# verlab/accelerated_features

Measured on AMD Instinct MI355X. Metric: frames/sec detectAndCompute+match (VGA, top_k=4096), higher is better.
Workload: dtype f32; 1 GPU; VGA 640x480 sparse top_k=4096, batch=64 per GPU: detectAndCompute + MNN match of the 32 consecutive frame pairs (BASELINE configs[1]); batch_per_gpu=64, height=480, width=640, top_k=4096, weights=synthetic (tests/fixtures.py), barrier=none (one rank), concurrent_lanes=True, lanes=2

## Files before the change

accelerated_features_amd/_lib.py:

```python
import ctypes as C
import os

_HERE = os.path.dirname(os.path.abspath(__file__))
LIB_PATH = os.environ.get("XFH_LIB_PATH") or os.path.join(_HERE, "libxfeat_hip.so")

XFH_OK = 0
LAYOUT_NCHW, LAYOUT_NHWC = 0, 1
LG_NO_PRUNING = 1 << 30
GUIDE_FUNDAMENTAL, GUIDE_HOMOGRAPHY = 0, 1
SAMPLE_MODES = {'nearest': 0, 'bilinear': 1, 'bicubic': 2}
PROF_NONE, PROF_CONV_MFMA, PROF_MATCH, PROF_BLOCK1, PROF_HEADS, PROF_CONV_64_64_S1, PROF_CONV_24_24, PROF_CONV_LAYER0 = 0, 1, 2, 3, 4, 5, 6, 100
PROF_ALL = 1000

_p = C.c_void_p
_i = C.c_int
_f = C.c_float
_sz = C.c_size_t
SIGNATURES = {
    "xfh_version": (_i, []),
    "xfh_last_error": (C.c_char_p, []),
    "xfh_num_weight_arrays": (_i, []),
    "xfh_weight_array_floats": (_sz, [_i]),
    "xfh_create": (_i, [C.POINTER(_p), _i, _i, C.POINTER(_p)]),
    "xfh_destroy": (None, [_p]),
    "xfh_resize_bilinear": (_i, [_p, _i, _i, _i, _p, _i, _i, _f, _f, _p]),
    "xfh_backbone_workspace_bytes": (_sz, [_i, _i, _i, _i]),
    "xfh_backbone": (_i, [_p, _p, _i, _i, _i, _i, _p, _p, _p, _p, _p, _p, _sz, _p]),
    "xfh_backbone_u8": (_i, [_p, _p, _i, _f, _i, _i, _i, _i, _p, _p, _p, _p, _p, _p, _sz, _p]),
    "xfh_backbone_resized": (_i, [_p, _p, _i, _i, _i, _i, _i, _i, _f, _f, _i, _i, _f, _f, _p, _p, _p, _p, _p, _p, _sz, _p]),
    "xfh_conv_layer": (_i, [_p, _i, _p, _i, _i, _i, _p, _i, _p]),
    "xfh_detect_workspace_bytes": (_sz, [_i, _i, _i, _i, _i]),
    "xfh_detect_sparse": (_i, [_p, _p, _p, _p, _p, _i, _i, _i, _f, _i, _i, _f, _f, _p, _p, _p, _p, _p, _p, _p, _sz, _p]),
    "xfh_dense_workspace_bytes": (_sz, [_i, _i, _i, _i]),
    "xfh_extract_dense": (_i, [_p, _p, _p, _i, _i, _i, _i, _f, _f, _f, _p, _p, _p, _p, _sz, _p]),
    "xfh_match_workspace_bytes": (_sz, [_i, _i, _i]),
# ... 107 lines not shown
```

accelerated_features_amd/csrc/api.hip:

```cpp
#include "../../include/xfeat_hip.h"
#include "kernels.hpp"
#include "weight_split.hpp"
#include "block1_fx.hpp"

#include <cmath>
#include <cstdarg>
#include <cstdio>
#include <cstring>
#include <vector>

using namespace xfh;

static thread_local char g_err[512] = "";
static int fail(int code, const char* fmt, ...) {
    va_list ap;
    va_start(ap, fmt);
    vsnprintf(g_err, sizeof(g_err), fmt, ap);
    va_end(ap);
    return code;
}
int xfh_set_error(int code, const char* fmt, ...) {
    char buf[512];
    va_list ap;
    va_start(ap, fmt);
// ... 222 lines not shown

int xfh_version(void) { return XFH_VERSION; }
const char* xfh_last_error(void) { return g_err; }
int xfh_num_weight_arrays(void) { return num_arrays(); }
size_t xfh_weight_array_floats(int i) { return array_floats(i); }

int xfh_create(const float* const* host_arrays, int n_arrays, int device, xfh_handle* out) {
    if (!host_arrays || !out) return fail(XFH_ERR_ARG, "xfh_create: NULL argument");
    if (n_arrays != num_arrays()) return fail(XFH_ERR_WEIGHTS, "xfh_create: expected %d weight arrays, got %d", num_arrays(), n_arrays);
    for (int i = 0; i < n_arrays; ++i)
        if (!host_arrays[i]) return fail(XFH_ERR_WEIGHTS, "xfh_create: weight array %d is NULL", i);
    int ndev = 0;
    if (hipGetDeviceCount(&ndev) != hipSuccess || ndev <= 0) return fail(XFH_ERR_DEVICE, "xfh_create: no HIP device visible");
    if (device < 0 || device >= ndev) return fail(XFH_ERR_DEVICE, "xfh_create: device %d out of range (%d visible)", device, ndev);
    hipDeviceProp_t prop;
    HIP_TRY(hipGetDeviceProperties(&prop, device));
    if (strncmp(prop.gcnArchName, "gfx950", 6) != 0)
        return fail(XFH_ERR_DEVICE, "xfh_create: device %d is %s; this library is built for gfx950 only", device, prop.gcnArchName);
    HIP_TRY(hipSetDevice(device));

    std::vector<float> blob;
    auto reserve = [&](size_t n) { size_t o = align_up(blob.size(), 64); blob.resize(o + n, 0.f); return o; };
    const size_t zoff = reserve(256);
    struct Off { size_t oihw, kc, kcp, bias, fx, rs; bool has_fx, has_rs; } coff[L_NUM];
    struct FOff { size_t w, b, fx; bool fx_ok; } foff[5];
    int ai = 0;
    for (int li = 0; li < L_NUM; ++li) {
        const ConvSpec& c = kConvs[li];
        const int kk = c.ks * c.ks, cpad = (c.cout + 31) / 32 * 32;
        const float* w = host_arrays[ai++];
        std::vector<double> scale(c.cout, 1.0), shift(c.cout, 0.0);
        if (c.bn) {
            const float* rm = host_arrays[ai++];
            const float* rv = host_arrays[ai++];
            for (int o = 0; o < c.cout; ++o) {
                if (!(rv[o] + kBnEps > 0)) return fail(XFH_ERR_WEIGHTS, "layer %d: running_var[%d] = %g is not positive", li, o, rv[o]);
                scale[o] = 1.0 / std::sqrt((double)rv[o] + kBnEps);
                shift[o] = -(double)rm[o] * scale[o];
            }
        } else {
            const float* b = host_arrays[ai++];
            for (int o = 0; o < c.cout; ++o) shift[o] = b[o];
        }
        coff[li].oihw = reserve((size_t)c.cout * c.cin * kk);
        coff[li].kc = reserve((size_t)c.cin * kk * c.cout);
        coff[li].kcp = reserve((size_t)c.cin * kk * cpad);
        coff[li].bias = reserve(cpad);
// ... 34 lines not shown
                    for (int lane = 0; lane < 64; ++lane) {
                        const int o = lane & 31, kg = 2 * st + (lane >> 5);
                        for (int i = 0; i < 8; ++i) {
                            float v = 0.f;
                            if (o < c.cout && kg < 9 * cg) v = blob[coff[li].oihw + ((size_t)o * c.cin + (kg % cg) * 8 + i) * 9 + kg / cg];
                            split_weight(v, q);
                            for (int sp = 0; sp < 3; ++sp) dst[(((size_t)st * 3 + sp) * 64 + lane) * 8 + i] = q[sp];
                        }
                    }
            if (bx24s2)
                for (int cb = 0; cb < 2; ++cb)
                    for (int st = 0; st < nstep; ++st)
                        for (int lane = 0; lane < 64; ++lane) {
                            const int o = cb * 32 + (lane & 31), kg = 2 * st + (lane >> 5);
                            for (int i = 0; i < 8; ++i) {
                                float v = 0.f;
                                if (kg < 9 * cg) v = blob[coff[li].oihw + ((size_t)o * c.cin + (kg % cg) * 8 + i) * 9 + kg / cg];
                                split_weight(v, q);
                                for (int sp = 0; sp < 3; ++sp) dst[((((size_t)cb * nstep + st) * 3 + sp) * 64 + lane) * 8 + i] = q[sp];
                            }
                        }
            if (bx64s2) pack_bx64(&blob[coff[li].oihw], c.cin, c.cout, dst);
        }
        coff[li].has_rs = false;
        if (bx1x1 && fx_ok) {
            coff[li].rs = reserve((size_t)4 * 2 * 3 * 64 * 4);
            pack_rs64_1x1(&blob[coff[li].oihw], reinterpret_cast<uint16_t*>(&blob[coff[li].rs]));
            coff[li].has_rs = true;
        }
        if (bx128 && fx_ok) {
            coff[li].rs = reserve(4 * kRs64Halfs / 2);
            pack_rs128(&blob[coff[li].oihw], reinterpret_cast<uint16_t*>(&blob[coff[li].rs]));
            coff[li].has_rs = true;
        }
        if (bx64 && fx_ok) {
            coff[li].rs = reserve(kRs64Halfs / 2);
            pack_rs64(&blob[coff[li].oihw], reinterpret_cast<uint16_t*>(&blob[coff[li].rs]));
            coff[li].has_rs = true;
        }
    }
    size_t head_off[2] = {0, 0}, head_boff[2] = {0, 0};
    bool head_fx_ok[2] = {true, true};
    const float head_b_last = blob[coff[L_HEAT_2].bias];
    {
        const int kp[4] = {L_KP_0, L_KP_1, L_KP_2, L_KP_3}, rel[2] = {L_HEAT_0, L_HEAT_1};
        for (int hd = 0; hd < 2; ++hd) {
// ... 65 lines not shown
            pack_linear_fx(wk.data(), f.k, npad, reinterpret_cast<uint16_t*>(blob.data() + foff[fi].fx));
        }
    }

    xfh_context* ctx = new xfh_context();
    ctx->device = device;
    ctx->blob = nullptr;
    hipError_t e = hipMalloc((void**)&ctx->blob, blob.size() * sizeof(float));
    if (e == hipSuccess) e = hipMemcpy(ctx->blob, blob.data(), blob.size() * sizeof(float), hipMemcpyHostToDevice);
    if (e != hipSuccess) {
        if (ctx->blob) (void)hipFree(ctx->blob);
        delete ctx;
        return fail(XFH_ERR_HIP, "xfh_create: weight upload failed: %s", hipGetErrorString(e));
    }
    for (int li = 0; li < L_NUM; ++li) {
        const ConvSpec& c = kConvs[li];
        ConvW& w = ctx->nw.conv[li];
        w.cin = c.cin; w.cout = c.cout; w.ks = c.ks; w.stride = c.stride; w.relu = c.bn; w.cout_pad = (c.cout + 31) / 32 * 32;
        w.w_oihw = ctx->blob + coff[li].oihw;
        w.w_kc = ctx->blob + coff[li].kc;
        w.w_kcp = ctx->blob + coff[li].kcp;
        w.bias = ctx->blob + coff[li].bias;
        w.w_fx = coff[li].has_fx ? ctx->blob + coff[li].fx : nullptr;
        w.w_rs = coff[li].has_rs ? ctx->blob + coff[li].rs : nullptr;
    }
    ctx->nw.zeros = ctx->blob + zoff;
    for (int hd = 0; hd < 2; ++hd) {
        ctx->nw.head_fx[hd] = head_fx_ok[hd] ? ctx->blob + head_off[hd] : nullptr;
        ctx->nw.head_bx_bias[hd] = ctx->blob + head_boff[hd];
    }
    ctx->nw.block1_fx = b1fx_ok ? ctx->blob + b1fx_off : nullptr;
    ctx->nw.block1_fx3 = b1fx_ok ? ctx->blob + b1fx3_off : nullptr;
    ctx->nw.head_rel_b_last = head_b_last;
    ctx->nw.head_kp_b_dust = blob[coff[L_KP_3].bias + 64];
    for (int fi = 0; fi < 5; ++fi) {
        LinW& l = ctx->nw.fine[fi];
        l.k = kFine[fi].k; l.n = kFine[fi].n; l.n_pad = (kFine[fi].n + 63) / 64 * 64; l.relu = kFine[fi].bn;
        l.w_kn = ctx->blob + foff[fi].w;
        l.bias = ctx->blob + foff[fi].b;
        l.w_fx = foff[fi].fx_ok ? ctx->blob + foff[fi].fx : nullptr;
    }
    *out = ctx;
    return XFH_OK;
}

void xfh_destroy(xfh_handle h) {
// ... 25 lines not shown
    if (B <= 0 || H <= 0 || W <= 0) return 0;
    BackboneWs o;
    return carve_backbone(nullptr, B, H, W, o);
}

static int conv_mfma_checked(xfh_handle h, int layer, int fused_layer, const float* in, int B, int Hin, int Win, float* out,
                             bool nhwc, hipStream_t st, bool in_backbone = false, int link = 0) {
    const ConvW& c = h->nw.conv[layer];
    const ConvW* c2 = fused_layer >= 0 ? &h->nw.conv[fused_layer] : nullptr;
    const int pad = c.ks / 2;
    const int Hout = (Hin + 2 * pad - c.ks) / c.stride + 1, Wout = (Win + 2 * pad - c.ks) / c.stride + 1;
    int pid = h->prof.which >= 100 ? 100 + layer : XFH_PROF_CONV_MFMA;
    if (h->prof.which == XFH_PROF_CONV_64_64_S1 && c.cin == 64 && c.cout == 64 && c.ks == 3 && c.stride == 1) pid = XFH_PROF_CONV_64_64_S1;
    if (h->prof.which == XFH_PROF_CONV_24_24 && c.cin == 24 && c.cout == 24 && c.ks == 3 && c.stride == 1) pid = XFH_PROF_CONV_24_24;
    prof_begin(&h->prof, pid, st);
    int rc = -1;
    const int fx = h->opt.fx;
    if ((fx & XFH_FX_CONV64) && c.ks == 3 && c.stride == 1 && c.w_rs) {
        if (c.cin == 64 && !c2 && !nhwc) rc = launch_conv_rs64(c, in, B, Hin, Win, out, st, h->status, nullptr, false, h->trace);
        else if (c.cin == 128 && !c2 && !nhwc) rc = launch_conv_rs128(c, in, B, Hin, Win, out, st, h->status);
        else if (c.cin == 64 && c2 && c2->w_rs) rc = launch_conv_rs64(c, in, B, Hin, Win, out, st, h->status, c2, nhwc, h->trace);
    }
    if (rc && (fx & XFH_FX_CONV64) && c.w_fx && !c2 && !nhwc && c.stride == 2 && c.cin == 64) rc = launch_conv_bx64s2_fx(c, in, B, Hin, Win, out, st, h->trace, h->status);
    if (rc && (fx & XFH_FX_CONV24) && c.w_fx && !c2 && !nhwc && c.cin == 24) rc = launch_conv_bx(c, in, B, Hin, Win, out, st, h->trace, h->status, link & 1, (link & 2) != 0);
    if (rc && link) return fail(XFH_ERR_UNSUPPORTED, "layer %d: a channels-last link without its fp16-pair kernel", layer);
    if (rc) rc = launch_conv_mfma(c, c2, h->nw.zeros, in, B, Hin, Win, out, nhwc, st, h->trace);
    const int cl = c2 ? c2->cout : c.cout;
    double bytes = 4.0 * ((double)B * c.cin * Hin * Win + (double)B * cl * Hout * Wout + (double)c.cin * c.cout * c.ks * c.ks);
    double flops = conv_flops(c, B, Hout, Wout);
    if (c2) { flops += conv_flops(*c2, B, Hout, Wout); bytes += 4.0 * c2->cin * c2->cout; }
    prof_end(&h->prof, pid, st, flops, bytes);
    if (rc) return fail(XFH_ERR_UNSUPPORTED, "no MFMA conv instantiation for layer %d (%d->%d k%d s%d) at %dx%d", layer, c.cin, c.cout, c.ks, c.stride, Hin, Win);
    return XFH_OK;
}

struct ResizeSpec { int Hin, Win, Hm, Wm; float s1h, s1w, s2h, s2w; };

static int backbone_impl(xfh_handle h, const float* img, const unsigned char* img_u8, int u8_layout, float u8_divisor, int B, int C, int H,
                         int W, float* feats, float* logits, float* heat, float* reliab, float* invnorm, void* workspace, size_t workspace_bytes,
                         xfh_stream stream, const ResizeSpec* rs = nullptr) {
    if (!h || (!img && !img_u8) || !feats || !reliab) return fail(XFH_ERR_ARG, "xfh_backbone: NULL argument");
    if (!logits && !heat) return fail(XFH_ERR_ARG, "xfh_backbone: logits and heat are both NULL");
    int rc = check_img("xfh_backbone", B, C, H, W);
    if (rc) return rc;
    BackboneWs w;
    const size_t need = carve_backbone(workspace, B, H, W, w);
// ... 70 lines not shown
    return backbone_impl(h, nullptr, img, layout, divisor, B, C, H, W, feats, logits, heat, reliab, invnorm, workspace, workspace_bytes, stream);
}

int xfh_backbone_resized(xfh_handle h, const float* img, int B, int C, int Hin, int Win, int Hmid, int Wmid, float scale1_h, float scale1_w,
                         int Hout, int Wout, float scale2_h, float scale2_w, float* feats, float* logits, float* heat, float* reliab, float* invnorm,
                         void* workspace, size_t workspace_bytes, xfh_stream stream) {
    if (Hin <= 0 || Win <= 0 || Hmid <= 0 || Wmid <= 0 || !(scale1_h > 0.f) || !(scale1_w > 0.f))
        return fail(XFH_ERR_ARG, "xfh_backbone_resized: bad source / intermediate size");
    const ResizeSpec rs{Hin, Win, Hmid, Wmid, scale1_h, scale1_w, scale2_h, scale2_w};
    return backbone_impl(h, img, nullptr, 0, 1.f, B, C, Hout, Wout, feats, logits, heat, reliab, invnorm, workspace, workspace_bytes, stream, &rs);
}

int xfh_conv_layer(xfh_handle h, int layer, const float* in, int B, int Hin, int Win, float* out, int variant,
                   xfh_stream stream) {
    if (!h || !in || !out) return fail(XFH_ERR_ARG, "xfh_conv_layer: NULL argument");
    if (layer < 0 || layer >= L_NUM) return fail(XFH_ERR_ARG, "xfh_conv_layer: layer %d out of range", layer);
    if (B <= 0 || Hin <= 0 || Win <= 0 || B > 4000) return fail(XFH_ERR_ARG, "xfh_conv_layer: bad shape");
    hipStream_t st = (hipStream_t)stream;
    const ConvW& c = h->nw.conv[layer];
    if (variant == XFH_CONV_VARIANT_GENERIC) {
        launch_conv_generic(c, in, B, Hin, Win, out, st);
        return check_launch("xfh_conv_layer(generic)");
    }
    if (variant == XFH_CONV_VARIANT_FX) {
        int rc = -1;
        if (c.ks == 3 && c.cin == 24) rc = launch_conv_bx(c, in, B, Hin, Win, out, st, h->trace, h->status);
        else if (c.ks == 3 && c.cin == 64 && c.stride == 2) rc = launch_conv_bx64s2_fx(c, in, B, Hin, Win, out, st, h->trace, h->status);
        else if (c.ks == 3 && c.cin == 64 && c.stride == 1 && c.w_rs) rc = launch_conv_rs64(c, in, B, Hin, Win, out, st, h->status, nullptr, false, h->trace);
        else if (c.ks == 3 && c.cin == 128 && c.stride == 1 && c.w_rs) rc = launch_conv_rs128(c, in, B, Hin, Win, out, st, h->status);
        if (rc) return fail(XFH_ERR_UNSUPPORTED, "xfh_conv_layer: no fp16-pair kernel for layer %d at %dx%d", layer, Hin, Win);
        return check_launch("xfh_conv_layer(fp16 pair)");
    }
    if (variant == XFH_CONV_VARIANT_FX_PAIR || variant == XFH_CONV_VARIANT_FX_PAIR_NHWC) {
        if (layer + 1 >= L_NUM) return fail(XFH_ERR_ARG, "xfh_conv_layer: layer %d has no successor", layer);
        const ConvW& c2 = h->nw.conv[layer + 1];
        if (c2.ks != 1 || c2.cin != 64 || c2.cout != 64 || c.cin != 64 || c.ks != 3 || c.stride != 1 || !c.w_rs || !c2.w_rs ||
            launch_conv_rs64(c, in, B, Hin, Win, out, st, h->status, &c2, variant == XFH_CONV_VARIANT_FX_PAIR_NHWC, nullptr))
            return fail(XFH_ERR_UNSUPPORTED, "xfh_conv_layer: no fused 3x3 + 1x1 kernel for layers %d, %d at width %d", layer, layer + 1, Win);
        return check_launch("xfh_conv_layer(3x3 + 1x1)");
    }
    if (variant == XFH_CONV_VARIANT_F32) {
        if (launch_conv_mfma(c, nullptr, h->nw.zeros, in, B, Hin, Win, out, false, st, h->trace))
            return fail(XFH_ERR_UNSUPPORTED, "xfh_conv_layer: no f32-MFMA kernel for layer %d at %dx%d", layer, Hin, Win);
        return check_launch("xfh_conv_layer(f32 mfma)");
    }
    if (variant != 0) return fail(XFH_ERR_ARG, "xfh_conv_layer: unknown variant %d", variant);
    if (layer >= L_BLOCK1_0 && layer <= L_BLOCK1_3) {
        launch_block1_layer(h->nw, layer, in, B, Hin, Win, out, st);
        return check_launch("xfh_conv_layer(block1)");
// ... 897 lines not shown
```

accelerated_features_amd/csrc/kernels.hpp:

```cpp
#pragma once
#include "common.hpp"

namespace xfh {

constexpr int GS_CHUNKS = 64;

enum Layer {
    L_SKIP1 = 0, L_BLOCK1_0, L_BLOCK1_1, L_BLOCK1_2, L_BLOCK1_3, L_BLOCK2_0, L_BLOCK2_1,
    L_BLOCK3_0, L_BLOCK3_1, L_BLOCK3_2, L_BLOCK4_0, L_BLOCK4_1, L_BLOCK4_2,
    L_BLOCK5_0, L_BLOCK5_1, L_BLOCK5_2, L_BLOCK5_3, L_FUSION_0, L_FUSION_1, L_FUSION_2,
    L_HEAT_0, L_HEAT_1, L_HEAT_2, L_KP_0, L_KP_1, L_KP_2, L_KP_3, L_NUM
};

struct ConvW {
    int cin, cout, ks, stride, relu, cout_pad;
    const float* w_oihw;
    const float* w_kc;
    const float* w_kcp;
    const float* bias;
    const void* w_fx;
    const void* w_rs;
};

struct LinW {
    int k, n, n_pad, relu;
    const float* w_kn;
    const float* bias;
    const void* w_fx;
};

struct NetWeights {
    ConvW conv[L_NUM];
    LinW fine[5];
    const float* zeros;
    const void* head_fx[2];
    const float* head_bx_bias[2];
    float head_rel_b_last;
    float head_kp_b_dust;
    const void* block1_fx;
    const void* block1_fx3;
};

struct Profiler;
// ... 9 lines not shown

void launch_gray_norm(const float* img, int B, int C, int H, int W, double* part, float* gray, float* coef, hipStream_t st);
int launch_gray_norm_resized(const float* img, int B, int C, int Hin, int Win, int Hm, int Wm, float s1h, float s1w, int Ho, int Wo,
                             float s2h, float s2w, double* part, float* gray, float* coef, hipStream_t st, int form = 1);
void launch_gray_norm_u8(const unsigned char* img, bool nhwc, float divisor, int B, int C, int H, int W, double* part, float* gray,
                         float* coef, hipStream_t st);
void launch_resize_bilinear(const float* src, int planes, int Hin, int Win, float* dst, int Hout, int Wout,
                            float sh, float sw, hipStream_t st);
int launch_pyramid53(const ConvW& c53, const float* x3, const float* x4, const float* y5, float* out, int B,
                     int H3, int W3, int H4, int W4, int H5, int W5, hipStream_t st);
void launch_pyramid_sum(const float* x3, const float* x4, const float* x5, float* out, int planes,
                        int H3, int W3, int H4, int W4, int H5, int W5, hipStream_t st);

void launch_block1(const NetWeights& nw, const float* gray, int B, int H, int W, float* t0, float* t1, float* t2,
                   float* x1, hipStream_t st);
void launch_block1_fused(const NetWeights& nw, const float* gray, const float* coef, int B, int H, int W, float* x1, hipStream_t st, int variant = 7, int* status = nullptr);
int launch_block1_layer(const NetWeights& nw, int layer, const float* in, int B, int Hin, int Win, float* out,
                        hipStream_t st);
void launch_conv_generic(const ConvW& c, const float* in, int B, int Hin, int Win, float* out, hipStream_t st);

int launch_conv_mfma(const ConvW& c, const ConvW* fused1x1, const float* zeros, const float* in, int B, int Hin, int Win,
                     float* out, bool nhwc_out, hipStream_t st, long long* trace = nullptr);
int launch_conv_bx(const ConvW& c, const float* in, int B, int H, int W, float* out, hipStream_t st, long long* trace = nullptr, int* status = nullptr, bool in_cl = false, bool out_cl = false);
bool conv_bx_links(const ConvW& c, bool tracing);
int launch_conv_rs64(const ConvW& c, const float* in, int B, int H, int W, float* out, hipStream_t st, int* status = nullptr, const ConvW* fused1x1 = nullptr, bool nhwc = false,
                     long long* trace = nullptr);
bool conv_rs128_fits(int W);
int launch_conv_rs128(const ConvW& c, const float* in, int B, int H, int W, float* out, hipStream_t st, int* status = nullptr);
int launch_conv_bx64s2_fx(const ConvW& c, const float* in, int B, int H, int W, float* out, hipStream_t st, long long* trace = nullptr, int* status = nullptr);
int bx_steps(int cin);
size_t homography_workspace_bytes(int P, int max_iters);
void launch_homography_tables(double thr, unsigned* stab, double* wtab, hipStream_t st);
int launch_find_homography(const float* p0, const float* p1, const int64_t* idx0, const int64_t* idx1, int kcap, const int32_t* counts, int n_const, int P, int cap, double thr, int max_iters,
                           double confidence, unsigned long long seed, double* H, unsigned char* mask, int32_t* info, void* ws, hipStream_t st);
size_t relpose_workspace_bytes(int P, int max_iters);
int launch_estimate_relpose(const float* p0, const float* p1, const int64_t* idx0, const int64_t* idx1, int kcap, const int32_t* counts, int n_const,
                            int P, int cap, const double* K0, const double* K1, double max_err, int min_iters, int max_iters, double success_prob,
                            unsigned long long seed, double* R, double* t, double* E, unsigned char* mask, int32_t* info, void* ws, hipStream_t st);
size_t relpose_sweep_workspace_bytes(int P, int max_iters, int T);
int launch_estimate_relpose_sweep(const float* p0, const float* p1, const int64_t* idx0, const int64_t* idx1, int kcap, const int32_t* counts, int n_const,
                                  int P, int cap, const double* K0, const double* K1, const double* max_errs, int T, int min_iters, int max_iters,
                                  double success_prob, unsigned long long seed, double* R, double* t, double* E, unsigned char* mask, int32_t* info,
                                  void* ws, hipStream_t st);
size_t abspose_workspace_bytes(int P, int max_iters);
int launch_estimate_abspose(const float* p2, const float* p3, const int64_t* idx2, const int64_t* idx3, int cap2, int cap3, const int32_t* counts,
                            int n_const, int P, int cap, const double* K, double max_err, int min_iters, int max_iters, double success_prob,
// ... 164 lines not shown
```

accelerated_features_amd/csrc/weight_split.hpp:

```cpp
#pragma once
#include <cstdint>
#include <cstring>

namespace xfh {

inline uint16_t f16_rne(float f) {
    uint32_t u;
    memcpy(&u, &f, 4);
    const uint32_t sign = (u >> 16) & 0x8000u;
    u &= 0x7fffffffu;
    if (u >= 0x7f800000u) return (uint16_t)(sign | (u > 0x7f800000u ? 0x7e00u : 0x7c00u));
    if (u >= 0x477ff000u) return (uint16_t)(sign | 0x7c00u);
    if (u < 0x38800000u) {
        if (u < 0x33000000u) return (uint16_t)sign;
        const int e = (int)(u >> 23);
        const uint32_t m = (u & 0x7fffffu) | 0x800000u;
        const int sh = 126 - e;
        const uint32_t q = m >> sh, rem = m & ((1u << sh) - 1u), halfway = 1u << (sh - 1);
        return (uint16_t)(sign | (q + ((rem > halfway || (rem == halfway && (q & 1u))) ? 1u : 0u)));
    }
    const uint32_t v = u - 0x38000000u;
    return (uint16_t)(sign | ((v + 0xfffu + ((v >> 13) & 1u)) >> 13));
}
inline float f16_float(uint16_t h) {
// ... 81 lines not shown
        for (int wv = 0; wv < 4; ++wv)
            for (int tap = 0; tap < 9; ++tap)
                for (int ck = 0; ck < 2; ++ck)
                    for (int lane = 0; lane < 64; ++lane)
                        for (int i = 0; i < 8; ++i) {
                            const int o = cq * 32 + (lane & 31), ci = wv * 32 + ck * 16 + 8 * (lane >> 5) + i;
                            uint16_t q[3];
                            split_weight(w[((size_t)o * 128 + ci) * 9 + tap], q);
                            for (int sp = 0; sp < 3; ++sp) dst[(((((((size_t)cq * 4 + wv) * 9 + tap) * 2 + ck) * 3 + sp) * 64) + lane) * 8 + i] = q[sp];
                        }
    return 4 * kRs64Halfs;
}
inline size_t pack_rs64_1x1(const float* w, uint16_t* dst) {
    for (int wv = 0; wv < 4; ++wv)
        for (int s = 0; s < 2; ++s)
            for (int lane = 0; lane < 64; ++lane)
                for (int i = 0; i < 8; ++i) {
                    uint16_t q[3];
                    split_weight(w[(size_t)(16 * wv + (lane & 15)) * 64 + 32 * s + 8 * (lane >> 4) + i], q);
                    for (int sp = 0; sp < 3; ++sp) dst[((((size_t)wv * 2 + s) * 3 + sp) * 64 + lane) * 8 + i] = q[sp];
                }
    return (size_t)4 * 2 * 3 * 64 * 8;
}
}
```

include/xfeat_hip.h:

```cpp
#ifndef XFEAT_HIP_H
#define XFEAT_HIP_H

#include <stddef.h>
#include <stdint.h>

#ifdef __cplusplus
extern "C" {
#endif

#define XFH_VERSION 303

enum {
    XFH_OK = 0,
    XFH_ERR_ARG = -1,
    XFH_ERR_WEIGHTS = -2,
    XFH_ERR_WORKSPACE = -3,
    XFH_ERR_UNSUPPORTED = -4,
    XFH_ERR_HIP = -5,
    XFH_ERR_DEVICE = -6
};

typedef struct xfh_context* xfh_handle;
typedef void* xfh_stream;

// ... 10 lines not shown

enum { XFH_FX_CONV64 = 1, XFH_FX_CONV24 = 2, XFH_FX_HEADS = 8, XFH_FX_FINE = 2048, XFH_FX_ALL = 1 | 2 | 8 | 2048 };
int xfh_set_option(xfh_handle h, const char* key, int value);
int xfh_get_option(xfh_handle h, const char* key, int* value);
enum { XFH_STATUS_FX_RANGE = 1 };
int xfh_set_status_buffer(xfh_handle h, int32_t* device_word);

size_t xfh_backbone_workspace_bytes(int B, int C, int H, int W);
int xfh_backbone(xfh_handle h, const float* img, int B, int C, int H, int W,
                 float* feats, float* logits, float* heat, float* reliab, float* invnorm,
                 void* workspace, size_t workspace_bytes, xfh_stream stream);

#define XFH_LAYOUT_NCHW 0
#define XFH_LAYOUT_NHWC 1
int xfh_backbone_u8(xfh_handle h, const uint8_t* img, int layout, float divisor, int B, int C, int H, int W,
                    float* feats, float* logits, float* heat, float* reliab, float* invnorm,
                    void* workspace, size_t workspace_bytes, xfh_stream stream);

int xfh_backbone_resized(xfh_handle h, const float* img, int B, int C, int Hin, int Win, int Hmid, int Wmid,
                         float scale1_h, float scale1_w, int Hout, int Wout, float scale2_h, float scale2_w,
                         float* feats, float* logits, float* heat, float* reliab, float* invnorm, void* workspace,
                         size_t workspace_bytes, xfh_stream stream);

enum { XFH_CONV_VARIANT_DEFAULT = 0, XFH_CONV_VARIANT_GENERIC = 1, XFH_CONV_VARIANT_FX = 2, XFH_CONV_VARIANT_F32 = 3, XFH_CONV_VARIANT_FX_PAIR = 4, XFH_CONV_VARIANT_FX_PAIR_NHWC = 5 };
int xfh_conv_layer(xfh_handle h, int layer, const float* in, int B, int Hin, int Win, float* out,
                   int variant, xfh_stream stream);

size_t xfh_detect_workspace_bytes(int B, int H, int W, int top_k, int nms_capacity);
int xfh_detect_sparse(xfh_handle h, const float* heat, const float* reliab, const float* feats, const float* invnorm,
                      int B, int H, int W, float threshold, int top_k, int nms_capacity, float rw, float rh,
                      float* kpts, float* scores, float* desc, uint16_t* desc_f16, int32_t* n_valid, int32_t* n_candidates,
                      void* workspace, size_t workspace_bytes, xfh_stream stream);

size_t xfh_dense_workspace_bytes(int B, int h, int w, int k);
int xfh_extract_dense(xfh_handle h, const float* reliab, const float* feats, int B, int hc, int wc, int k,
                      float rw, float rh, float scale_div, float* kpts, float* desc, int32_t* cell_index,
                      void* workspace, size_t workspace_bytes, xfh_stream stream);

size_t xfh_match_workspace_bytes(int P, int N1, int N2);
int xfh_match_mnn(xfh_handle h , const float* d1, size_t pair_stride1, const float* d2, size_t pair_stride2,
                  const uint16_t* d1_f16, const uint16_t* d2_f16,
                  const int32_t* n1, const int32_t* n2, int n_stride, int n_offset2,
                  int P, int N1, int N2, float min_cossim,
                  int64_t* idx0, int64_t* idx1, int32_t* n_matches,
                  void* workspace, size_t workspace_bytes, xfh_stream stream);

#define XFH_GUIDE_FUNDAMENTAL 0
// ... 229 lines not shown
```

Before: 57110 frames/s.

## Add packed 24-channel 3x3 conv kernel using 16-row MFMA tiles with split-fp16

Adds a new persistent conv kernel for 24-in/24-out 3x3 stride-1 layers. It packs the 24 output rows into a 16-row tile plus 8 rows interleaved with the low split component, so fewer MFMA rows are wasted than with the 32-row padded kernel. Input tiles are double-buffered in LDS and the next tile's loads are overlapped with the MFMA loop. The default dispatch now prefers this kernel when it is not tracing, keeping the old kernel as a selectable variant. The cost is an extra packed weight blob and a more intricate accumulation, including a permlane swap to combine the high halves.

Result: no change. 57570 frames/s, median of 6 (+0.8%).

```diff
diff --git a/accelerated_features_amd/_lib.py b/accelerated_features_amd/_lib.py
--- a/accelerated_features_amd/_lib.py
+++ b/accelerated_features_amd/_lib.py
@@ -11,6 +11,7 @@
 SAMPLE_MODES = {'nearest': 0, 'bilinear': 1, 'bicubic': 2}
 PROF_NONE, PROF_CONV_MFMA, PROF_MATCH, PROF_BLOCK1, PROF_HEADS, PROF_CONV_64_64_S1, PROF_CONV_24_24, PROF_CONV_LAYER0 = 0, 1, 2, 3, 4, 5, 6, 100
 PROF_ALL = 1000
+CONV_VARIANT_DEFAULT, CONV_VARIANT_GENERIC, CONV_VARIANT_FX, CONV_VARIANT_F32, CONV_VARIANT_FX_PAIR, CONV_VARIANT_FX_PAIR_NHWC, CONV_VARIANT_FX_32ROW = 0, 1, 2, 3, 4, 5, 6
 
 _p = C.c_void_p
 _i = C.c_int
diff --git a/accelerated_features_amd/csrc/api.hip b/accelerated_features_amd/csrc/api.hip
--- a/accelerated_features_amd/csrc/api.hip
+++ b/accelerated_features_amd/csrc/api.hip
@@ -268,7 +268,7 @@
     std::vector<float> blob;
     auto reserve = [&](size_t n) { size_t o = align_up(blob.size(), 64); blob.resize(o + n, 0.f); return o; };
     const size_t zoff = reserve(256);
-    struct Off { size_t oihw, kc, kcp, bias, fx, rs; bool has_fx, has_rs; } coff[L_NUM];
+    struct Off { size_t oihw, kc, kcp, bias, fx, fxp, rs; bool has_fx, has_fxp, has_rs; } coff[L_NUM];
     struct FOff { size_t w, b, fx; bool fx_ok; } foff[5];
     int ai = 0;
     for (int li = 0; li < L_NUM; ++li) {
@@ -349,6 +349,11 @@
                         }
             if (bx64s2) pack_bx64(&blob[coff[li].oihw], c.cin, c.cout, dst);
         }
+        coff[li].has_fxp = coff[li].has_fx && bx24 && c.cout == 24;
+        if (coff[li].has_fxp) {
+            coff[li].fxp = reserve(kBxpHalfs / 2);
+            pack_bxp(&blob[coff[li].oihw], reinterpret_cast<uint16_t*>(&blob[coff[li].fxp]));
+        }
         coff[li].has_rs = false;
         if (bx1x1 && fx_ok) {
             coff[li].rs = reserve((size_t)4 * 2 * 3 * 64 * 4);
@@ -460,6 +465,7 @@
         w.w_kcp = ctx->blob + coff[li].kcp;
         w.bias = ctx->blob + coff[li].bias;
         w.w_fx = coff[li].has_fx ? ctx->blob + coff[li].fx : nullptr;
+        w.w_fxp = coff[li].has_fxp ? ctx->blob + coff[li].fxp : nullptr;
         w.w_rs = coff[li].has_rs ? ctx->blob + coff[li].rs : nullptr;
     }
     ctx->nw.zeros = ctx->blob + zoff;
@@ -531,6 +537,7 @@
         else if (c.cin == 64 && c2 && c2->w_rs) rc = launch_conv_rs64(c, in, B, Hin, Win, out, st, h->status, c2, nhwc, h->trace);
     }
     if (rc && (fx & XFH_FX_CONV64) && c.w_fx && !c2 && !nhwc && c.stride == 2 && c.cin == 64) rc = launch_conv_bx64s2_fx(c, in, B, Hin, Win, out, st, h->trace, h->status);
+    if (rc && (fx & XFH_FX_CONV24) && c.w_fxp && !c2 && !nhwc && !h->trace) rc = launch_conv_bxp(c, in, B, Hin, Win, out, st, h->status, link & 1, (link & 2) != 0);
     if (rc && (fx & XFH_FX_CONV24) && c.w_fx && !c2 && !nhwc && c.cin == 24) rc = launch_conv_bx(c, in, B, Hin, Win, out, st, h->trace, h->status, link & 1, (link & 2) != 0);
     if (rc && link) return fail(XFH_ERR_UNSUPPORTED, "layer %d: a channels-last link without its fp16-pair kernel", layer);
     if (rc) rc = launch_conv_mfma(c, c2, h->nw.zeros, in, B, Hin, Win, out, nhwc, st, h->trace);
@@ -647,9 +654,12 @@
         launch_conv_generic(c, in, B, Hin, Win, out, st);
         return check_launch("xfh_conv_layer(generic)");
     }
-    if (variant == XFH_CONV_VARIANT_FX) {
+    if (variant == XFH_CONV_VARIANT_FX || variant == XFH_CONV_VARIANT_FX_32ROW) {
         int rc = -1;
-        if (c.ks == 3 && c.cin == 24) rc = launch_conv_bx(c, in, B, Hin, Win, out, st, h->trace, h->status);
+        if (variant == XFH_CONV_VARIANT_FX_32ROW) {
+            if (c.ks == 3 && c.cin == 24 && c.cout == 24 && c.stride == 1) rc = launch_conv_bx(c, in, B, Hin, Win, out, st, nullptr, h->status);
+        } else if (c.ks == 3 && c.cin == 24 && c.cout == 24 && c.stride == 1 && !h->trace) rc = launch_conv_bxp(c, in, B, Hin, Win, out, st, h->status);
+        else if (c.ks == 3 && c.cin == 24) rc = launch_conv_bx(c, in, B, Hin, Win, out, st, h->trace, h->status);
         else if (c.ks == 3 && c.cin == 64 && c.stride == 2) rc = launch_conv_bx64s2_fx(c, in, B, Hin, Win, out, st, h->trace, h->status);
         else if (c.ks == 3 && c.cin == 64 && c.stride == 1 && c.w_rs) rc = launch_conv_rs64(c, in, B, Hin, Win, out, st, h->status, nullptr, false, h->trace);
         else if (c.ks == 3 && c.cin == 128 && c.stride == 1 && c.w_rs) rc = launch_conv_rs128(c, in, B, Hin, Win, out, st, h->status);
diff --git a/accelerated_features_amd/csrc/conv_bxp_body.hpp b/accelerated_features_amd/csrc/conv_bxp_body.hpp
--- /dev/null
+++ b/accelerated_features_amd/csrc/conv_bxp_body.hpp
@@ -0,0 +1,254 @@
+#pragma once
+#ifndef XFH_HOST_EMU
+#include "kernels.hpp"
+#ifndef XFH_DYN_LDS_BYTES
+#define XFH_DYN_LDS_BYTES(name) extern __shared__ __attribute__((aligned(16))) unsigned char name[]
+#endif
+#ifndef XFH_PIN
+#define XFH_PIN(x) asm volatile("" : "+v"(x))
+#endif
+#define XFH_BXP_IDLE(a0, a1, a2, a3, a4, a5, a6, a7) asm volatile("s_nop 7\n\ts_nop 7" : "+v"(a0), "+v"(a1), "+v"(a2), "+v"(a3), "+v"(a4), "+v"(a5), "+v"(a6), "+v"(a7))
+#else
+#define XFH_BXP_IDLE(a0, a1, a2, a3, a4, a5, a6, a7) ((void)0)
+#endif
+#include "bx_split.hpp"
+
+namespace xfh {
+
+struct BxpArgs {
+    const float* in;
+    const uint4* wfrag;
+    const float* bias;
+    float* out;
+    int relu, H, W, B, tiles_x, tiles;
+    int cold;
+    int* status;
+};
+
+struct BxpCfg {
+    static constexpr int CIN = 24, COUT = 24;
+    static constexpr int TH = 16, TW = 32, IH = TH + 2, IW = TW + 2, NPIX = IH * IW;
+    static constexpr int NXS = 2;
+    static constexpr int CG = CIN / 8, SPLB = CIN * 2, PIXB = ((NXS * SPLB / 16) | 1) * 16;
+    static constexpr int KG = 9 * CG, NSTEP = (KG + 3) / 4, NHALF = 2 * NSTEP;
+    static constexpr int NITEM = NPIX * CG, NIT = (NITEM + 511) / 512;
+    static constexpr int TILE_BYTES = NPIX * PIXB;
+    static constexpr int BIAS_OFF = 2 * TILE_BYTES, LDS_BYTES = BIAS_OFF + 32 * 4;
+    static_assert(NIT == 4 && NHALF == 14 && LDS_BYTES <= 160 * 1024, "four staging items in fourteen half-steps, one CU's LDS");
+    static constexpr int koff(int kg) {
+        const int g = kg < KG ? kg : KG - 1;
+        const int tap = g / CG, cg = g % CG;
+        return ((tap / 3) * IW + tap % 3) * PIXB + cg * 16;
+    }
+};
+static_assert(BxpCfg::TILE_BYTES + ((BxpCfg::TH - 1) * BxpCfg::IW + 15) * BxpCfg::PIXB + BxpCfg::koff(BxpCfg::KG - 1) + 16 * BxpCfg::PIXB + BxpCfg::SPLB + 16 <= 2 * BxpCfg::TILE_BYTES,
+              "operand reads stay inside the tile buffers");
+
+typedef float f32x4 __attribute__((ext_vector_type(4)));
+
+template <bool IN_CL, bool OUT_CL>
+__device__ __forceinline__ void conv_bxp_body(const BxpArgs& a) {
+    using Cfg = BxpCfg;
+    using frag_t = f16x8;
+    auto mfma = [](frag_t x, frag_t y, f32x4 c) __attribute__((always_inline)) { return __builtin_amdgcn_mfma_f32_16x16x32_f16(x, y, c, 0, 0, 0); };
+    constexpr int CIN = Cfg::CIN, COUT = Cfg::COUT, TH = Cfg::TH, TW = Cfg::TW, IW = Cfg::IW, NPIX = Cfg::NPIX, PIXB = Cfg::PIXB, SPLB = Cfg::SPLB;
+    constexpr int NSTEP = Cfg::NSTEP, NHALF = Cfg::NHALF, NIT = Cfg::NIT, TILE_BYTES = Cfg::TILE_BYTES;
+    XFH_DYN_LDS_BYTES(smem_bp);
+    const int tid = threadIdx.x, lane = tid & 63, l15 = lane & 15, kq = lane >> 4;
+    const int wave = __builtin_amdgcn_readfirstlane(tid >> 6);
+    const size_t HW = (size_t)a.H * a.W;
+
+    frag_t w0[NSTEP], w2[NSTEP], wh[NSTEP];
+#pragma unroll
+    for (int s = 0; s < NSTEP; ++s) {
+        w0[s] = __builtin_bit_cast(frag_t, a.wfrag[(s * 3 + 0) * 64 + lane]);
+        w2[s] = __builtin_bit_cast(frag_t, a.wfrag[(s * 3 + 1) * 64 + lane]);
+        wh[s] = __builtin_bit_cast(frag_t, a.wfrag[(s * 3 + 2) * 64 + lane]);
+    }
+#pragma unroll
+    for (int s = 0; s < NSTEP; ++s) { XFH_PIN(w0[s]); XFH_PIN(w2[s]); XFH_PIN(wh[s]); }
+    _Float16 fz = l15 < 8 ? (_Float16)0.00048828125f : (_Float16)0.f;
+    float* bias_lds = reinterpret_cast<float*>(smem_bp + Cfg::BIAS_OFF);
+    if (tid < 32) bias_lds[tid] = a.bias[tid];
+
+    int it_rc[NIT], it_lds[NIT];
+#pragma unroll
+    for (int i = 0; i < NIT; ++i) {
+        int item = tid + 512 * i;
+        item = item >= Cfg::NITEM ? item - Cfg::NITEM : item;
+        const int cg = IN_CL ? item % Cfg::CG : item / NPIX, pix = IN_CL ? item / Cfg::CG : item - cg * NPIX;
+        const int r = pix / IW, c = pix - r * IW;
+        it_rc[i] = (cg << 16) | (r << 8) | c;
+        it_lds[i] = pix * PIXB + cg * 16;
+    }
+    unsigned pbase[NSTEP];
+#pragma unroll
+    for (int s = 0; s < NSTEP; ++s) {
+        const int kg = 4 * s + kq, g = kg < Cfg::KG ? kg : Cfg::KG - 1, tap = g / Cfg::CG, cg = g - tap * Cfg::CG, ty = tap / 3, tx = tap - 3 * ty;
+        pbase[s] = (unsigned)((2 * wave * IW + l15) * PIXB + (ty * IW + tx) * PIXB + cg * 16);
+    }
+    const int total = a.tiles * a.B;
+
+    auto tile_of = [&](int vid, int& b, int& oy0, int& ox0) {
+        int tile;
+        xcd_group_map(vid, a.tiles, a.B, b, tile);
+        const int tyi = tile / a.tiles_x, txi = tile - tyi * a.tiles_x;
+        oy0 = tyi * TH; ox0 = txi * TW;
+    };
+    unsigned amax = 0;
+    struct TileSrc { __amdgpu_buffer_rsrc_t rs; int oy0, ox0, live; };
+    auto src_of = [&](int vid) {
+        TileSrc t;
+        int b = 0, oy0 = 0, ox0 = 0;
+        t.live = vid < total;
+        if (t.live) tile_of(vid, b, oy0, ox0);
+        t.oy0 = oy0; t.ox0 = ox0;
+        t.rs = __builtin_amdgcn_make_buffer_rsrc((void*)(a.in + (size_t)b * CIN * HW), 0, (int)(CIN * HW * sizeof(float)), 0x00020000);
+        return t;
+    };
+    auto issue_item = [&](const TileSrc& t, int i, float (&v)[8]) __attribute__((always_inline)) {
+        const int cg = it_rc[i] >> 16, gy = t.oy0 - 1 + ((it_rc[i] >> 8) & 0xff), gx = t.ox0 - 1 + (it_rc[i] & 0xff);
+        const bool ok = (bool)((int)(t.live != 0) & (int)((unsigned)gy < (unsigned)a.H) & (int)((unsigned)gx < (unsigned)a.W));
+        if constexpr (IN_CL) {
+            const int voff = ok ? (int)((((size_t)gy * a.W + gx) * CIN + cg * 8) * 4) : (int)0x80000000;
+            const uint4 lo = __builtin_bit_cast(uint4, __builtin_amdgcn_raw_buffer_load_b128(t.rs, voff, 0, 0)), hi = __builtin_bit_cast(uint4, __builtin_amdgcn_raw_buffer_load_b128(t.rs, voff, 16, 0));
+            v[0] = __uint_as_float(lo.x); v[1] = __uint_as_float(lo.y); v[2] = __uint_as_float(lo.z); v[3] = __uint_as_float(lo.w);
+            v[4] = __uint_as_float(hi.x); v[5] = __uint_as_float(hi.y); v[6] = __uint_as_float(hi.z); v[7] = __uint_as_float(hi.w);
+        } else {
+            const int voff = ok ? (int)((((size_t)cg * 8) * HW + (size_t)gy * a.W + gx) * 4) : (int)0x80000000;
+#pragma unroll
+            for (int k = 0; k < 8; ++k) v[k] = __uint_as_float(__builtin_amdgcn_raw_buffer_load_b32(t.rs, voff, (int)(k * HW * 4), 0));
+        }
+    };
+    auto stage_item = [&](unsigned char* buf, int i, const float (&v)[8]) __attribute__((always_inline)) {
+        uint4 h, l;
+        split2_f16(v[0], v[1], h.x, l.x); split2_f16(v[2], v[3], h.y, l.y);
+        split2_f16(v[4], v[5], h.z, l.z); split2_f16(v[6], v[7], h.w, l.w);
+        fx_track_h(amax, h.x, true); fx_track_h(amax, h.y, true); fx_track_h(amax, h.z, true); fx_track_h(amax, h.w, true);
+        unsigned char* p = buf + it_lds[i];
+        *reinterpret_cast<uint4*>(p) = h;
+        *reinterpret_cast<uint4*>(p + SPLB) = l;
+    };
+
+    int vid = blockIdx.x;
+    if (vid >= total) return;
+    float va[8], vb[8];
+    {
+        const TileSrc t0 = src_of(vid);
+        issue_item(t0, 0, va); issue_item(t0, 1, vb);
+        stage_item(smem_bp, 0, va); issue_item(t0, 2, va);
+        stage_item(smem_bp, 1, vb); issue_item(t0, 3, vb);
+        stage_item(smem_bp, 2, va); stage_item(smem_bp, 3, vb);
+    }
+    __syncthreads();
+    int cur = 0;
+    for (;;) {
+        int b, oy0, ox0;
+        tile_of(vid, b, oy0, ox0);
+        unsigned char* nb = smem_bp + (cur ^ 1) * TILE_BYTES;
+        const TileSrc t1 = src_of(vid + (int)gridDim.x);
+#pragma unroll
+        for (int s = 0; s < NSTEP; ++s) XFH_PIN(pbase[s]);
+        f32x4 lo[2][2], hi[2][2];
+#pragma unroll
+        for (int j = 0; j < 2; ++j)
+#pragma unroll
+            for (int p = 0; p < 2; ++p)
+#pragma unroll
+                for (int r = 0; r < 4; ++r) { lo[j][p][r] = 0.f; hi[j][p][r] = 0.f; }
+        struct Frag { frag_t x[2][2]; };
+        Frag f[2];
+        auto load = [&](int h, Frag& o) __attribute__((always_inline)) {
+            const unsigned char* p = smem_bp + pbase[h >> 1] + (h & 1) * IW * PIXB;
+#pragma unroll
+            for (int pb = 0; pb < 2; ++pb)
+#pragma unroll
+                for (int q = 0; q < 2; ++q) o.x[pb][q] = *reinterpret_cast<const frag_t*>(p + pb * 16 * PIXB + q * SPLB);
+        };
+        load(0, f[0]);
+        frag_t a1, al;
+#pragma unroll
+        for (int h = 0; h < NHALF; ++h) {
+            const int s = h >> 1, j = h & 1;
+            const Frag& c = f[h & 1];
+            if (h + 1 < NHALF) load(h + 1, f[(h + 1) & 1]);
+            if (j == 0) {
+                XFH_PIN(w0[s]); XFH_PIN(wh[s]);
+                a1 = w0[s] * (_Float16)0.00048828125f;
+                al = wh[s] * fz;
+                XFH_PIN(a1); XFH_PIN(al);
+            }
+            const frag_t a0 = w0[s], a2 = w2[s], ah = wh[s];
+            __builtin_amdgcn_sched_barrier(0);
+#define BXP_MM(ACC, A, Q) { ACC[j][0] = mfma(A, c.x[0][Q], ACC[j][0]); ACC[j][1] = mfma(A, c.x[1][Q], ACC[j][1]); }
+            BXP_MM(lo, a2, 0) BXP_MM(hi, ah, 0) BXP_MM(lo, a1, 1) BXP_MM(hi, al, 1) BXP_MM(lo, a0, 0)
+#undef BXP_MM
+            __builtin_amdgcn_sched_barrier(0);
+            if (h == 0) issue_item(t1, 0, va);
+            if (h == 3) issue_item(t1, 1, vb);
+            if (h == 5) stage_item(nb, 0, va);
+            if (h == 6) issue_item(t1, 2, va);
+            if (h == 8) stage_item(nb, 1, vb);
+            if (h == 9) issue_item(t1, 3, vb);
+            if (h == 11) stage_item(nb, 2, va);
+            if (h == 13) stage_item(nb, 3, vb);
+            __builtin_amdgcn_sched_barrier(0);
+        }
+        XFH_BXP_IDLE(lo[0][0], lo[0][1], lo[1][0], lo[1][1], hi[0][0], hi[0][1], hi[1][0], hi[1][1]);
+        __builtin_amdgcn_sched_barrier(0);
+        const float4 bl = *reinterpret_cast<const float4*>(bias_lds + 4 * kq), bh = *reinterpret_cast<const float4*>(bias_lds + 16 + 4 * (kq & 1));
+        const float bls[4] = {bl.x, bl.y, bl.z, bl.w}, bhs[4] = {bh.x, bh.y, bh.z, bh.w};
+        const __amdgpu_buffer_rsrc_t rs_out = __builtin_amdgcn_make_buffer_rsrc((void*)(a.out + (size_t)b * COUT * HW), 0, (int)(COUT * HW * sizeof(float)), 0x00020000);
+        typedef unsigned u32x4s __attribute__((ext_vector_type(4)));
+#pragma unroll
+        for (int j = 0; j < 2; ++j) {
+            const int oy = oy0 + 2 * wave + j;
+            float yh[4];
+#pragma unroll
+            for (int r = 0; r < 4; ++r) {
+                const auto sw = __builtin_amdgcn_permlane32_swap(__float_as_uint(hi[j][0][r]), __float_as_uint(hi[j][1][r]), false, false);
+                yh[r] = fmaf(__uint_as_float(sw[0]) + __uint_as_float(sw[1]), FX_SCALE_INV, bhs[r]);
+                if (a.relu) yh[r] = fmaxf(yh[r], 0.f);
+            }
+            const int oxh = ox0 + 16 * (lane >> 5) + l15, ch = 16 + 4 * (kq & 1);
+            const bool okh = oy < a.H && oxh < a.W;
+            if constexpr (OUT_CL) {
+                const u32x4s u = {__float_as_uint(yh[0]), __float_as_uint(yh[1]), __float_as_uint(yh[2]), __float_as_uint(yh[3])};
+                __builtin_amdgcn_raw_buffer_store_b128(u, rs_out, okh ? (int)((((size_t)oy * a.W + oxh) * COUT + ch) * 4) : (int)0x80000000, 0, 0);
+            } else {
+                const int voff = okh ? (int)(((size_t)ch * HW + (size_t)oy * a.W + oxh) * 4) : (int)0x80000000;
+#pragma unroll
+                for (int r = 0; r < 4; ++r) __builtin_amdgcn_raw_buffer_store_b32(__float_as_uint(yh[r]), rs_out, voff, (int)(r * HW * 4), 0);
+            }
+#pragma unroll
+            for (int p = 0; p < 2; ++p) {
+                const int ox = ox0 + 16 * p + l15;
+                const bool ok = oy < a.H && ox < a.W;
+                float y[4];
+#pragma unroll
+                for (int r = 0; r < 4; ++r) {
+                    y[r] = fmaf(lo[j][p][r], FX_SCALE_INV, bls[r]);
+                    if (a.relu) y[r] = fmaxf(y[r], 0.f);
+                }
+                if constexpr (OUT_CL) {
+                    const u32x4s u = {__float_as_uint(y[0]), __float_as_uint(y[1]), __float_as_uint(y[2]), __float_as_uint(y[3])};
+                    __builtin_amdgcn_raw_buffer_store_b128(u, rs_out, ok ? (int)((((size_t)oy * a.W + ox) * COUT + 4 * kq) * 4) : (int)0x80000000, 0, 0);
+                } else {
+                    const int voff = ok ? (int)(((size_t)(4 * kq) * HW + (size_t)oy * a.W + ox) * 4) : (int)0x80000000;
+#pragma unroll
+                    for (int r = 0; r < 4; ++r) __builtin_amdgcn_raw_buffer_store_b32(__float_as_uint(y[r]), rs_out, voff, (int)(r * HW * 4), 0);
+                }
+            }
+        }
+        const int nvid = vid + (int)gridDim.x;
+        if (nvid >= total) break;
+        __syncthreads();
+        vid = nvid;
+#pragma unroll
+        for (int s = 0; s < NSTEP; ++s) pbase[s] += cur ? 0u - (unsigned)TILE_BYTES : (unsigned)TILE_BYTES;
+        cur ^= 1;
+    }
+    fx_report_h(amax, a.status);
+}
+
+}
diff --git a/accelerated_features_amd/csrc/k_conv_bxp.hip b/accelerated_features_amd/csrc/k_conv_bxp.hip
--- /dev/null
+++ b/accelerated_features_amd/csrc/k_conv_bxp.hip
@@ -0,0 +1,38 @@
+#include "kernels.hpp"
+#include "conv_bxp_body.hpp"
+
+namespace xfh {
+
+template <bool IN_CL, bool OUT_CL>
+__global__ __launch_bounds__(512) __attribute__((amdgpu_waves_per_eu(2, 2)))
+void conv_bxp_kernel(BxpArgs a) {
+    kernel_entry_hooks(a.cold);
+    conv_bxp_body<IN_CL, OUT_CL>(a);
+}
+
+template <bool IN_CL, bool OUT_CL>
+static int run_bxp(const ConvW& c, const float* in, int B, int H, int W, float* out, hipStream_t st, int* status) {
+    using Cfg = BxpCfg;
+    if ((size_t)Cfg::CIN * H * W * sizeof(float) >= 0x7fffffffu) return -1;
+    BxpArgs a;
+    a.cold = g_debug_cold;
+    a.status = status;
+    a.in = in; a.wfrag = reinterpret_cast<const uint4*>(c.w_fxp); a.bias = c.bias; a.out = out; a.relu = c.relu; a.H = H; a.W = W; a.B = B;
+    a.tiles_x = ceil_div(W, Cfg::TW);
+    a.tiles = a.tiles_x * ceil_div(H, Cfg::TH);
+    static AttrMask attr_done = 0;
+    set_max_dynamic_lds(reinterpret_cast<const void*>(conv_bxp_kernel<IN_CL, OUT_CL>), Cfg::LDS_BYTES, attr_done);
+    const int total = xcd_grid_size(a.tiles, B);
+    int grid = num_cus();
+    if (grid > total) grid = total;
+    conv_bxp_kernel<IN_CL, OUT_CL><<<grid, 512, Cfg::LDS_BYTES, st>>>(a);
+    return 0;
+}
+
+int launch_conv_bxp(const ConvW& c, const float* in, int B, int H, int W, float* out, hipStream_t st, int* status, bool in_cl, bool out_cl) {
+    if (c.ks != 3 || c.stride != 1 || c.cin != 24 || c.cout != 24 || !c.w_fxp) return -1;
+    if (in_cl) return out_cl ? run_bxp<true, true>(c, in, B, H, W, out, st, status) : -1;
+    return out_cl ? run_bxp<false, true>(c, in, B, H, W, out, st, status) : run_bxp<false, false>(c, in, B, H, W, out, st, status);
+}
+
+}
diff --git a/accelerated_features_amd/csrc/kernels.hpp b/accelerated_features_amd/csrc/kernels.hpp
--- a/accelerated_features_amd/csrc/kernels.hpp
+++ b/accelerated_features_amd/csrc/kernels.hpp
@@ -19,6 +19,7 @@
     const float* w_kcp;
     const float* bias;
     const void* w_fx;
+    const void* w_fxp;
     const void* w_rs;
 };
 
@@ -74,6 +75,7 @@
 int launch_conv_mfma(const ConvW& c, const ConvW* fused1x1, const float* zeros, const float* in, int B, int Hin, int Win,
                      float* out, bool nhwc_out, hipStream_t st, long long* trace = nullptr);
 int launch_conv_bx(const ConvW& c, const float* in, int B, int H, int W, float* out, hipStream_t st, long long* trace = nullptr, int* status = nullptr, bool in_cl = false, bool out_cl = false);
+int launch_conv_bxp(const ConvW& c, const float* in, int B, int H, int W, float* out, hipStream_t st, int* status = nullptr, bool in_cl = false, bool out_cl = false);
 bool conv_bx_links(const ConvW& c, bool tracing);
 int launch_conv_rs64(const ConvW& c, const float* in, int B, int H, int W, float* out, hipStream_t st, int* status = nullptr, const ConvW* fused1x1 = nullptr, bool nhwc = false,
                      long long* trace = nullptr);
diff --git a/accelerated_features_amd/csrc/weight_split.hpp b/accelerated_features_amd/csrc/weight_split.hpp
--- a/accelerated_features_amd/csrc/weight_split.hpp
+++ b/accelerated_features_amd/csrc/weight_split.hpp
@@ -127,4 +127,23 @@
                 }
     return (size_t)4 * 2 * 3 * 64 * 8;
 }
+constexpr size_t kBxpHalfs = (size_t)7 * 3 * 64 * 8;
+inline size_t pack_bxp(const float* w, uint16_t* dst) {
+    for (int st = 0; st < 7; ++st)
+        for (int lane = 0; lane < 64; ++lane) {
+            const int row = lane & 15, kg = 4 * st + (lane >> 4);
+            for (int i = 0; i < 8; ++i) {
+                uint16_t lo[3] = {0, 0, 0}, hi[3] = {0, 0, 0};
+                if (kg < 27) {
+                    split_weight(w[((size_t)row * 24 + (kg % 3) * 8 + i) * 9 + kg / 3], lo);
+                    split_weight(w[((size_t)(16 + (row & 7)) * 24 + (kg % 3) * 8 + i) * 9 + kg / 3], hi);
+                }
+                uint16_t* d = dst + ((size_t)st * 3 * 64 + lane) * 8 + i;
+                d[0] = lo[0];
+                d[64 * 8] = lo[2];
+                d[2 * 64 * 8] = row < 8 ? hi[0] : hi[2];
+            }
+        }
+    return kBxpHalfs;
 }
+}
diff --git a/include/xfeat_hip.h b/include/xfeat_hip.h
--- a/include/xfeat_hip.h
+++ b/include/xfeat_hip.h
@@ -56,7 +56,8 @@
                          float* feats, float* logits, float* heat, float* reliab, float* invnorm, void* workspace,
                          size_t workspace_bytes, xfh_stream stream);
 
-enum { XFH_CONV_VARIANT_DEFAULT = 0, XFH_CONV_VARIANT_GENERIC = 1, XFH_CONV_VARIANT_FX = 2, XFH_CONV_VARIANT_F32 = 3, XFH_CONV_VARIANT_FX_PAIR = 4, XFH_CONV_VARIANT_FX_PAIR_NHWC = 5 };
+enum { XFH_CONV_VARIANT_DEFAULT = 0, XFH_CONV_VARIANT_GENERIC = 1, XFH_CONV_VARIANT_FX = 2, XFH_CONV_VARIANT_F32 = 3, XFH_CONV_VARIANT_FX_PAIR = 4, XFH_CONV_VARIANT_FX_PAIR_NHWC = 5,
+       XFH_CONV_VARIANT_FX_32ROW = 6 };
 int xfh_conv_layer(xfh_handle h, int layer, const float* in, int B, int Hin, int Win, float* out,
                    int variant, xfh_stream stream);
 
```
